# brucechin/OctopusZK

Hardware: AMD Instinct MI355X
Metric: BN254 G1 VariableBaseMSM Mscalar-mul/s at 2^20 (higher is better)
Workload: dtype u32; 1 GPU; VariableBaseMSM BN254 G1 2^20 random scalars/bases per GPU, bit-exact vs the serial CPU path (BASELINE.json configs[1]); n_per_gpu=1048576, window_bits=16, windows=8, glv=True, prepared_bases=False, msms_in_flight=3, schedule=pipeline3, parallelism=index-range shard x1, RCCL all-gather of 192-B partials + HIP point sum

## Files before the change

### octopuszk_amd/csrc/glv.cuh

```cuda
#pragma once
#include "curve.cuh"

namespace ozk {

struct GlvConsts {
  static constexpr u32 R32[8] = {0xf0000001u, 0x43e1f593u, 0x79b97091u, 0x2833e848u, 0x8181585du, 0xb85045b6u, 0xe131a029u, 0x30644e72u};
  static constexpr u32 G1C[3] = {0xc7e0b3d7u, 0xd91d232eu, 0x00000002u};
  static constexpr u32 G2C[5] = {0x391eb18du, 0x7a7bd9d4u, 0xa773d2cfu, 0x4ccef014u, 0x00000002u};
  static constexpr u32 A1[2] = {0x94d213e3u, 0x89d32568u};
  static constexpr u32 A2[4] = {0x1221250bu, 0x0be4e154u, 0xeeb859fdu, 0x6f4d8248u};
  static constexpr u32 B1ABS[4] = {0x7d4f1128u, 0x8211bbebu, 0xeeb859fcu, 0x6f4d8248u};
  static constexpr u32 B2[2] = {0x94d213e3u, 0x89d32568u};
  static constexpr u32 BETA_G1[9] = {0xa337995u, 0x158d1d23u, 0x189c9b98u, 0x12fa4e45u, 0x185faadcu, 0x176f16du, 0xeed93bau, 0x14291140u, 0xc0afeu};
  static constexpr u32 BETA_G2[9] = {0x18ccb791u, 0x175b1c3au, 0xb83d6e2u, 0xe8ed071u, 0x1282bee2u, 0x4220e84u, 0x1fe4017fu, 0x15084d4au, 0x169119u};
};

template <int NA, int NB, int NR>
OZK_HD void mp_mul_lo(const u32* a, const u32* b, u32* r) {
  u64 carry = 0;
#pragma unroll
  for (int k = 0; k < NR; k++) {
    u64 lo = carry & 0xffffffffull;
    u64 hi = carry >> 32;
#pragma unroll
    for (int i = 0; i < NA; i++) {
      const int j = k - i;
      if (j >= 0 && j < NB) {
        const u64 p = (u64)a[i] * b[j];
        lo += p & 0xffffffffull;
        hi += p >> 32;
      }
    }
    r[k] = (u32)lo;
    carry = hi + (lo >> 32);
  }
}
template <int NA, int NB>
OZK_HD void mp_mul(const u32* a, const u32* b, u32* r) { mp_mul_lo<NA, NB, NA + NB>(a, b, r); }

template <int N>
OZK_HD void mp_sub(u32* a, const u32* b) {
  u64 br = 0;
#pragma unroll
  for (int i = 0; i < N; i++) {
    const u64 t = (u64)a[i] - b[i] - br;
    a[i] = (u32)t;
    br = (t >> 32) & 1;
  }
}
template <int N>
OZK_HD bool mp_geq(const u32* a, const u32* b) {
  for (int i = N - 1; i >= 0; i--) {
    if (a[i] > b[i]) return true;
    if (a[i] < b[i]) return false;
  }
  return true;
}
template <int N>
OZK_HD void mp_neg(u32* a) {
  u64 c = 1;
#pragma unroll
  for (int i = 0; i < N; i++) {
    c += (u64)(~a[i]);
    a[i] = (u32)c;
    c >>= 32;
  }
}

OZK_HD void glv_decompose(const u32 (&k_in)[8], u32 (&k1)[4], bool& neg1, u32 (&k2)[4], bool& neg2) {
  u32 k[8];
#pragma unroll
  for (int i = 0; i < 8; i++) k[i] = k_in[i];
  for (int it = 0; it < 6 && mp_geq<8>(k, GlvConsts::R32); it++) mp_sub<8>(k, GlvConsts::R32);
  u32 p1[11], p2[13];
  mp_mul<8, 3>(k, GlvConsts::G1C, p1);
  mp_mul<8, 5>(k, GlvConsts::G2C, p2);
  const u32* c1 = p1 + 8;
  const u32* c2 = p2 + 8;
  u32 t1[5], t2[5], s1[5], s2[5];
  mp_mul_lo<3, 2, 5>(c1, GlvConsts::A1, t1);
  mp_mul_lo<5, 4, 5>(c2, GlvConsts::A2, t2);
#pragma unroll
  for (int i = 0; i < 5; i++) s1[i] = k[i];
  mp_sub<5>(s1, t1);
  mp_sub<5>(s1, t2);
  mp_mul_lo<3, 4, 5>(c1, GlvConsts::B1ABS, s2);
  mp_mul_lo<5, 2, 5>(c2, GlvConsts::B2, t2);
  mp_sub<5>(s2, t2);
  neg1 = (s1[4] >> 31) != 0;
  neg2 = (s2[4] >> 31) != 0;
  if (neg1) mp_neg<5>(s1);
  if (neg2) mp_neg<5>(s2);
#pragma unroll
  for (int i = 0; i < 4; i++) {
    k1[i] = s1[i];
    k2[i] = s2[i];
  }
}

template <class CV>
OZK_HD Fe<FqParams, 16> glv_beta() {
  if constexpr (CurveIO<CV>::CW == 16) return fe_const<FqParams, 16>(GlvConsts::BETA_G2);
  else return fe_const<FqParams, 16>(GlvConsts::BETA_G1);
}
template <class CV>
OZK_HD Aff<typename CV::EA> glv_image(const Aff<typename CV::EA>& q) {
  Aff<typename CV::EA> q2;
  q2.x = typename CV::EA(canonical(scale(q.x, glv_beta<CV>())));
  q2.y = q.y;
  return q2;
}

}
```

### octopuszk_amd/csrc/msm_var.cuh

```cuda
#pragma once
#include "curve.cuh"
#include "glv.cuh"

namespace ozk {

constexpr u32 BID_NONE = 0xffffffffu;

struct MsmPlan {
  int n_in;
  int glv;
  int n;
  int sd;
  int c;
  int cb;
  int W;
  int L1;
  int LK;
  int S;
};

OZK_HD u32 scalar_digit(const u32 (&s)[8], int w, int c) {
  const int bit = w * c;
  const int wi = bit >> 5, sh = bit & 31;
  u32 v = s[wi] >> sh;
  if (sh + c > 32 && wi + 1 < 8) v |= s[wi + 1] << (32 - sh);
  return v & ((1u << c) - 1u);
}

OZK_HD bool digit_decode(u32 code, int sd, u32& b, u32& neg) {
  if (sd) {
    const u32 t = code - 1u;
    b = t >> 1;
    neg = t & 1u;
  } else {
    b = code;
    neg = 0;
  }
  return code != 0;
}
template <class Emit>
OZK_HD void signed_digit_codes(const u32 (&e)[8], int c, int W, bool neg, Emit emit) {
  const u32 half = 1u << (c - 1);
  const u32 thr = (c == 16 && neg) ? half - 1u : half;
  u32 cy = 0;
  for (int w = 0; w < W; w++) {
    const u32 d = scalar_digit(e, w, c) + cy;
    cy = d > thr;
    const u32 m = cy ? (1u << c) - d : d;
    emit(w, (uint16_t)(m ? (((m - 1u) << 1) | (cy ^ (u32)neg)) + 1u : 0u));
  }
}

constexpr u32 SIDX_NEG = 0x80000000u;

#if defined(__HIPCC__)


template <class CV>
__global__ void __launch_bounds__(256) k_convert_bases(const u32* __restrict__ wire,
                                                       u32* __restrict__ aff, int n, int glv,
                                                       const uint8_t* __restrict__ neg_flags) {
  using IO = CurveIO<CV>;
  using EA = typename CV::EA;
  using ET = ElemTraits<EA>;
  const int i = blockIdx.x * blockDim.x + threadIdx.x;
  if (i >= n) return;
  const u32* p = wire + (size_t)i * IO::WIRE_JAC_WORDS;
  u32* o = aff + (size_t)i * IO::AFF_WORDS;
  Aff<EA> q;
  if (ET::wire_is_zero(p + 2 * IO::CW)) {
    q.x = EA(el_zero(q.x));
    q.y = EA(el_zero(q.x));
  } else if (ET::wire_is_one(p + 2 * IO::CW)) {
    q.x = ET::from_wire(p);
    q.y = ET::from_wire(p + IO::CW);
  } else {
    const EA X = ET::from_wire(p), Y = ET::from_wire(p + IO::CW), Z = ET::from_wire(p + 2 * IO::CW);
    const auto zi = inv(Z);
    if (is_zero(Z)) {
      q.x = EA(el_zero(q.x));
      q.y = EA(el_zero(q.x));
    } else {
      const auto zi2 = sqr(zi);
      q.x = EA(canonical(mul(X, zi2)));
      q.y = EA(canonical(mul(Y, mul(zi2, zi))));
    }
  }
  q.x = EA(canonical(q.x));
  q.y = EA(canonical(q.y));
  if (!glv) {
    IO::store_aff(q, o);
    return;
  }
  Aff<EA> q2;
  q2.x = EA(canonical(scale(q.x, glv_beta<CV>())));
  q2.y = q.y;
  if (neg_flags != nullptr) {
    const EA ny = EA(canonical(neg(q.y)));
    if (neg_flags[i]) q.y = ny;
    if (neg_flags[n + i]) q2.y = ny;
  }
  IO::store_aff(q, o);
  IO::store_aff(q2, aff + (size_t)(n + i) * IO::AFF_WORDS);
}

static __global__ void __launch_bounds__(256) k_digits(const u32* __restrict__ scalars, int n, int c, int W,
                                                uint16_t* __restrict__ digits) {
  const int i = blockIdx.x * blockDim.x + threadIdx.x;
  if (i >= n) return;
  u32 s[8];
  const uint4* sp = reinterpret_cast<const uint4*>(scalars + (size_t)i * 8);
  const uint4 a = sp[0], b = sp[1];
  s[0] = a.x; s[1] = a.y; s[2] = a.z; s[3] = a.w;
  s[4] = b.x; s[5] = b.y; s[6] = b.z; s[7] = b.w;
  for (int w = 0; w < W; w++) digits[(size_t)w * n + i] = (uint16_t)scalar_digit(s, w, c);
}

static __global__ void __launch_bounds__(256) k_digits_glv(const u32* __restrict__ scalars, int n, int c, int W, int sd,
                                                    uint16_t* __restrict__ digits, uint8_t* __restrict__ neg_flags) {
  const int i = blockIdx.x * blockDim.x + threadIdx.x;
  if (i >= n) return;
  u32 s[8];
  const uint4* sp = reinterpret_cast<const uint4*>(scalars + (size_t)i * 8);
  const uint4 a = sp[0], b = sp[1];
  s[0] = a.x; s[1] = a.y; s[2] = a.z; s[3] = a.w;
  s[4] = b.x; s[5] = b.y; s[6] = b.z; s[7] = b.w;
  u32 k1[4], k2[4];
  bool n1, n2;
  glv_decompose(s, k1, n1, k2, n2);
  u32 e1[8] = {k1[0], k1[1], k1[2], k1[3], 0, 0, 0, 0};
  u32 e2[8] = {k2[0], k2[1], k2[2], k2[3], 0, 0, 0, 0};
  const size_t ne = 2 * (size_t)n;
  if (sd) {
    signed_digit_codes(e1, c, W, n1, [&](int w, uint16_t code) { digits[(size_t)w * ne + i] = code; });
    signed_digit_codes(e2, c, W, n2, [&](int w, uint16_t code) { digits[(size_t)w * ne + n + i] = code; });
    return;
  } else {
    for (int w = 0; w < W; w++) {
      digits[(size_t)w * ne + i] = (uint16_t)scalar_digit(e1, w, c);
      digits[(size_t)w * ne + n + i] = (uint16_t)scalar_digit(e2, w, c);
    }
  }
  neg_flags[i] = n1;
  neg_flags[n + i] = n2;
}

constexpr int SORT_CHUNK = 4096;
constexpr int SORT_BLOCK = 256;

template <bool AGGREGATE = true>
__device__ __forceinline__ u32 lds_rank(u32* cnt, u32 key, bool live) {
  if constexpr (!AGGREGATE) return live ? atomicAdd(&cnt[key], 1u) : 0u;
  const unsigned long long m = __ballot(live);
  u32 r = 0;
  if (m != 0ull) {
    const int lane = threadIdx.x & 63;
    const int leader = __ffsll((long long)m) - 1;
    const u32 kl = __shfl(key, leader);
    if (__all(!live || key == kl)) {
      u32 base = 0;
      if (lane == leader) base = atomicAdd(&cnt[kl], (u32)__popcll(m));
      base = __shfl(base, leader);
      r = base + (u32)__popcll(m & ((1ull << lane) - 1ull));
    } else if (live) {
      r = atomicAdd(&cnt[key], 1u);
    }
  }
  return r;
}

static __global__ void __launch_bounds__(SORT_BLOCK) k_sort1_count(const uint16_t* __restrict__ digits, int n, int lo_bits,
                                                            int sd, int NH, int nblk, u32* __restrict__ C1) {
  extern __shared__ u32 cnt[];
  const int w = blockIdx.y, blk = blockIdx.x;
  for (int h = threadIdx.x; h < NH; h += SORT_BLOCK) cnt[h] = 0;
  block_sync();
  const int i0 = blk * SORT_CHUNK;
  constexpr int PER = SORT_CHUNK / SORT_BLOCK;
  u32 dreg[PER];
#pragma unroll
  for (int k = 0; k < PER; k++) {
    const int i = i0 + k * SORT_BLOCK + threadIdx.x;
    dreg[k] = (i < n) ? digits[(size_t)w * n + i] : 0u;
  }
#pragma unroll
  for (int k = 0; k < PER; k++) {
    u32 b, neg;
    const bool live = digit_decode(dreg[k], sd, b, neg);
    lds_rank(cnt, b >> lo_bits, live);
  }
  block_sync();
  for (int h = threadIdx.x; h < NH; h += SORT_BLOCK) C1[((size_t)w * NH + h) * nblk + blk] = cnt[h];
}

static __global__ void __launch_bounds__(SORT_BLOCK) k_sort1_scatter(const uint16_t* __restrict__ digits, int n, int lo_bits,
                                                              int sd, int NH, int nblk, const u32* __restrict__ P1,
                                                              const u32* __restrict__ total, size_t nC1,
                                                              u32* __restrict__ coarse) {
  extern __shared__ u32 sm[];
  u32* gdelta = sm;
  u32* lcur = sm + NH;
  u32* stage = sm + 2 * NH;
  u32* dest = stage + SORT_CHUNK;
  __shared__ u32 wsum[SORT_BLOCK / 64];
  __shared__ u32 n_local;
  const int w = blockIdx.y, blk = blockIdx.x;
  const int t = threadIdx.x;
  u32 g0 = 0, ct = 0;
  if (t < NH) {
    const size_t idx = ((size_t)w * NH + t) * nblk + blk;
    g0 = P1[idx];
    ct = ((idx + 1 < nC1) ? P1[idx + 1] : *total) - g0;
  }
  u32 incl = ct;
  const int lane = t & 63;
#pragma unroll
  for (int o = 1; o < 64; o <<= 1) {
    const u32 x = __shfl_up(incl, o);
    if (lane >= o) incl += x;
  }
// ... 733 lines not shown
        }
        cur = b;
        cur_cb = (p == s) && cb;
        if (b != BID_NONE) acc.start(pts_in, idx_in, p);
      } else if (b != BID_NONE) {
        acc.accumulate(pts_in, idx_in, p);
      }
    }
    }
    if (cur != BID_NONE) {
      if (cur_cb) {
        head_bid = cur;
        acc.store(pts_out + (size_t)(2 * (size_t)t) * IO::REC_WORDS);
        if (cf) {
          tail_bid = cur;
          if constexpr (FIRST) {
            acc.store_infinity(pts_out + (size_t)(2 * (size_t)t + 1) * IO::REC_WORDS);
          } else {
            IO::store_rec_jac(jac_infinity<CV>(), pts_out + (size_t)(2 * (size_t)t + 1) * IO::REC_WORDS);
          }
        }
      } else if (cf) {
        tail_bid = cur;
        acc.store(pts_out + (size_t)(2 * (size_t)t + 1) * IO::REC_WORDS);
      } else {
        acc.store(buckets + (size_t)cur * IO::REC_WORDS);
      }
    }
  }
  bid_out[2 * (size_t)t] = head_bid;
  bid_out[2 * (size_t)t + 1] = tail_bid;
}

template <class CV, bool FIRST, bool LAZY = false>
__global__ void __launch_bounds__(256, (FIRST && CV::LDS_ACC) ? 2 : 1)
k_segreduce(const u32* __restrict__ bid_in, const u32* __restrict__ idx_in, const u32* __restrict__ pts_in,
            const u32* __restrict__ d_count, int n_in_static, int L,
            u32* __restrict__ buckets, u32* __restrict__ bid_out, u32* __restrict__ pts_out,
            int n_lanes, unsigned long long* __restrict__ clk) {
  const int t = blockIdx.x * blockDim.x + threadIdx.x;
  unsigned long long w0 = 0, c0 = 0;
  if constexpr (FIRST) {
    if (clk != nullptr && threadIdx.x == 0) {
      w0 = (unsigned long long)wall_clock64();
      c0 = (unsigned long long)clock64();
      atomicMax(&clk[0], ~w0);
    }
  }
  if (t < n_lanes)
    segreduce_lane<CV, FIRST, LAZY>(t, bid_in, idx_in, pts_in, d_count, n_in_static, L, buckets, bid_out, pts_out);
  if constexpr (FIRST) {
    if (clk != nullptr && (threadIdx.x & 63) == 0) {
      const unsigned long long w1 = (unsigned long long)wall_clock64();
      atomicMax(&clk[1], w1);
      if (threadIdx.x == 0) {
        atomicAdd(&clk[2], (unsigned long long)clock64() - c0);
        atomicAdd(&clk[3], w1 - w0);
      }
    }
  }
}

static __global__ void k_read_clock(unsigned long long* out) { out[0] = (unsigned long long)wall_clock64(); }

template <class CV>
__global__ void __launch_bounds__(256)
k_segreduce_small(const u32* __restrict__ d_count, int n_in, int L, u32* __restrict__ buckets,
                  u32* __restrict__ bid_a, u32* __restrict__ pts_a, u32* __restrict__ bid_b, u32* __restrict__ pts_b) {
  if (*d_count == 0) return;
  u32 *bi = bid_a, *pi = pts_a, *bo = bid_b, *po = pts_b;
  while (true) {
    const int lanes = (n_in + L - 1) / L;
    for (int t = threadIdx.x; t < lanes; t += blockDim.x)
      segreduce_lane<CV, false>(t, bi, nullptr, pi, d_count, n_in, L, buckets, bo, po);
    if (lanes == 1) break;
    block_sync();
    n_in = 2 * lanes;
    u32* tb = bi; bi = bo; bo = tb;
    u32* tp = pi; pi = po; po = tp;
  }
}

constexpr int RUN_MAX = 16;
template <class CV>
__global__ void __launch_bounds__(256)
k_runmerge(const u32* __restrict__ bid_in, const u32* __restrict__ pts, int n_slots,
           u32* __restrict__ buckets, u32* __restrict__ bid_out, u32* __restrict__ remaining) {
  using IO = CurveIO<CV>;
  const int t = blockIdx.x * blockDim.x + threadIdx.x;
  u32 alive = 0;
#pragma unroll 1
  for (int k = 0; k < 2; k++) {
    const int x = 2 * t + 1 + k;
    if (x >= n_slots) break;
    const u32 bx = bid_in[x];
    u32 out = BID_NONE;
    if (bx != BID_NONE) {
      int s = x, e = x;
      while (s > 0 && x - s < RUN_MAX && bid_in[s - 1] == bx) s--;
      while (e + 1 < n_slots && e - x < RUN_MAX && bid_in[e + 1] == bx) e++;
      const bool is_short = (x - s < RUN_MAX) && (e - x < RUN_MAX) && (e - s + 1 <= RUN_MAX);
      if (!is_short) {
        out = bx;
      } else if (s == x) {
        Xyzz<CV> acc = IO::load_xyzz(pts + (size_t)s * IO::REC_WORDS);
        for (int q = s + 1; q <= e; q += 2) acc = xyzz_add(acc, IO::load_xyzz(pts + (size_t)q * IO::REC_WORDS));
        IO::store_rec_xyzz(acc, buckets + (size_t)bx * IO::REC_WORDS);
      }
    }
    bid_out[x] = out;
    alive += (out != BID_NONE);
  }
  if (t == 0 && n_slots > 0) {
    bid_out[0] = bid_in[0];
    alive += (bid_in[0] != BID_NONE);
  }
  for (int o = 32; o > 0; o >>= 1) alive += __shfl_xor(alive, o);
  if ((threadIdx.x & 63) == 0 && alive) atomicAdd(remaining, alive);
}

template <class CV, bool FIRSTLEVEL>
__global__ void __launch_bounds__(256)
k_wsum(const u32* __restrict__ A_in, const u32* __restrict__ R_in, const u32* __restrict__ hist,
       int m_in, int S, int g, u32* __restrict__ A_out, u32* __restrict__ R_out, int m_out, int W, int prio) {
  using IO = CurveIO<CV>;
  if (prio) __builtin_amdgcn_s_setprio(3);
  const int t = blockIdx.x * blockDim.x + threadIdx.x;
  if (t >= m_out * W) return;
  const int w = t / m_out, j = t - w * m_out;
  const size_t base = (size_t)w * m_in;
  const int lo = j * S;
  int hi = lo + S;
  if (hi > m_in) hi = m_in;
  Jac<CV> run = jac_infinity<CV>(), ws = jac_infinity<CV>(), asum = jac_infinity<CV>();
  for (int e = hi - 1; e >= lo; e--) {
    if constexpr (FIRSTLEVEL) {
      if (hist[base + e] != 0) run = jac_add(run, IO::load_rec(R_in + (base + e) * IO::REC_WORDS));
    } else {
      run = jac_add(run, IO::load_jac(R_in + (base + e) * IO::JAC_WORDS));
    }
    if (e > lo) ws = jac_add(ws, run);
    if constexpr (!FIRSTLEVEL) asum = jac_add(asum, IO::load_jac(A_in + (base + e) * IO::JAC_WORDS));
  }
  for (int k = 0; k < g; k++) ws = jac_dbl(ws);
  if constexpr (!FIRSTLEVEL) ws = jac_add(ws, asum);
  IO::store_jac(ws, A_out + ((size_t)w * m_out + j) * IO::JAC_WORDS);
  IO::store_jac(run, R_out + ((size_t)w * m_out + j) * IO::JAC_WORDS);
}

template <class CV>
__device__ __forceinline__ Jac<CV> shfl_down_jac(const Jac<CV>& p, int o) {
  Jac<CV> r;
  r.X = shfl_down_el(p.X, o);
  r.Y = shfl_down_el(p.Y, o);
  r.Z = shfl_down_el(p.Z, o);
  return r;
}

template <class CV>
__device__ __forceinline__ void wave_combine(Jac<CV>& A, Jac<CV>& T, int l, int valid, int g) {
  for (int o = 1; o < valid; o <<= 1) {
    const Jac<CV> t = shfl_down_jac(T, o);
    const Jac<CV> s = jac_add(T, t);
    if (l + o < 64) T = s;
  }
  Jac<CV> U = T;
  for (int k = 0; k < g; k++) U = jac_dbl(U);
  const Jac<CV> AV = jac_add(A, U);
  Jac<CV> V = (l >= 1) ? AV : A;
  int top = 1;
  while (top < valid) top <<= 1;
  for (int o = top >> 1; o > 0; o >>= 1) {
    const Jac<CV> v = shfl_down_jac(V, o);
    const Jac<CV> s = jac_add(V, v);
    if (l < o) V = s;
  }
  A = V;
}

template <class CV>
__global__ void __launch_bounds__(64)
k_wsum_wave(const u32* __restrict__ A_in, const u32* __restrict__ R_in, int m_in, int g,
            u32* __restrict__ A_out, u32* __restrict__ R_out, int m_out, int W) {
  using IO = CurveIO<CV>;
  __builtin_amdgcn_s_setprio(3);
  const int wave = blockIdx.x;
  if (wave >= m_out * W) return;
  const int w = wave / m_out, j = wave - w * m_out;
  const int l = threadIdx.x & 63;
  const int e = j * 64 + l;
  int valid = m_in - j * 64;
  if (valid > 64) valid = 64;
  Jac<CV> A = jac_infinity<CV>(), T = jac_infinity<CV>();
  if (e < m_in) {
    A = IO::load_jac(A_in + ((size_t)w * m_in + e) * IO::JAC_WORDS);
    T = IO::load_jac(R_in + ((size_t)w * m_in + e) * IO::JAC_WORDS);
  }
  wave_combine<CV>(A, T, l, valid, g);
  if (l == 0) {
    IO::store_jac(A, A_out + ((size_t)w * m_out + j) * IO::JAC_WORDS);
    IO::store_jac(T, R_out + ((size_t)w * m_out + j) * IO::JAC_WORDS);
// ... 220 lines not shown
```

### octopuszk_amd/csrc/msm_var_driver.cuh

```cuda
#pragma once
#include <hip/hip_ext.h>
#include <pthread.h>
#include <stdlib.h>

#include <atomic>
#include <vector>

#ifndef OZK_WITH_G2
#define OZK_WITH_G2 1
#endif
#include "msm_var.cuh"
#include "host_ctx.h"
#include "fq2.cuh"

namespace ozk {

enum { PROF_OFF = 0, PROF_EVENTS = 1, PROF_CLOCK = 2 };
struct ProfState {
  pthread_mutex_t mu = PTHREAD_MUTEX_INITIALIZER;
  std::atomic<int> mode{PROF_OFF};
  int src = PROF_EVENTS;
  int every = 1, seen = 0;
  int count = 0;
  std::vector<hipEvent_t> e0, e1;
// ... 212 lines not shown
}
template <class CV>
RegionBytes region_bytes(int n) {
  RegionBytes rb;
  make_layout3<CV>(plan_for<CV>(n), nullptr, nullptr, nullptr, &rb);
  return rb;
}

template <class CV>
size_t tail_layout(const MsmPlan& p, MsmLayout& L, void* tail, size_t tail_bytes) {
  using IO = CurveIO<CV>;
  Bump b(tail, tail_bytes);
  L.NB = (size_t)p.W << p.cb;
  L.m1 = (((size_t)1 << p.cb) + p.S - 1) / p.S;
  L.buckets = b.take<u32>(L.NB * IO::REC_WORDS);
  L.hist_t = b.take<u32>(L.NB);
  for (int k = 0; k < 2; k++) {
    L.wA[k] = b.take<u32>((size_t)p.W * L.m1 * IO::JAC_WORDS);
    L.wR[k] = b.take<u32>((size_t)p.W * L.m1 * IO::JAC_WORDS);
  }
  b.take<u32>(64);
  return b.off;
}

enum { TAIL_LATENCY = 0, TAIL_THROUGHPUT = 1 };
struct TailShape {
  bool fused;
  int serial_above;
};
static TailShape tail_shape(int mode) {
  const int forced = env_int("OZK_MSM_TAIL_MODE", -1);
  if (forced == 0 || forced == 1) mode = forced;
  TailShape t;
  t.fused = env_int("OZK_MSM_WSUM_FUSED", mode == TAIL_THROUGHPUT ? 0 : 1) != 0;
  t.serial_above = env_int("OZK_MSM_TAIL_SERIAL_ABOVE", mode == TAIL_THROUGHPUT ? 64 : (1 << 30));
  return t;
}
static void first_level_shape(const MsmPlan& p, bool fused, int* m_out, int* g_out) {
  const int m_in = 1 << p.cb;
  const int nseg = (m_in + p.S - 1) / p.S;
  const int sg = ilog2((uint32_t)p.S);
  if (fused) {
    *m_out = (nseg + 63) / 64;
    *g_out = sg + 6;
  } else {
    *m_out = nseg;
    *g_out = sg;
  }
}
template <class CV>
void launch_wsum0(const MsmPlan& p, const MsmLayout& L, hipStream_t st, int prio, bool fused) {
  const int TB = 256;
  const int m_in = 1 << p.cb;
  int m_out, g;
  first_level_shape(p, fused, &m_out, &g);
  const int tot = m_out * p.W;
  if (fused)
    hipLaunchKernelGGL((k_wsum_fused<CV>), dim3(tot), dim3(64), 0, st, L.buckets, L.hist_t, m_in, p.S,
                       ilog2((uint32_t)p.S), L.wA[0], L.wR[0], m_out, p.W, prio);
  else
    hipLaunchKernelGGL((k_wsum<CV, true>), dim3((tot + TB - 1) / TB), dim3(TB), 0, st, (const u32*)nullptr,
                       L.buckets, L.hist_t, m_in, p.S, 0, L.wA[0], L.wR[0], m_out, p.W, prio);
}

template <class CV>
int var_msm_sort(const void* d_bases, const void* d_scalars, int n, void* sorted, size_t sorted_bytes,
                        void* sort_ws, size_t sort_ws_bytes, hipStream_t st, hipEvent_t order_ev = nullptr,
                        const void* prepared = nullptr) {
  hip_clear_stale();
  const MsmPlan p = plan_for<CV>(n);
  if (prepared && p.glv && !p.sd) return fail(OZK_E_INVALID, "prepared bases need the signed-digit plan");
  RegionBytes rb;
  const MsmLayout L = make_layout3<CV>(p, sorted, sort_ws, nullptr, &rb, prepared);
  if (rb.sorted > sorted_bytes || rb.sort_ws > sort_ws_bytes)
    return fail(OZK_E_INVALID, "sort buffers too small: need %zu + %zu bytes, got %zu + %zu", rb.sorted, rb.sort_ws,
                sorted_bytes, sort_ws_bytes);
  const int TB = 256;
  const u32* bases = (const u32*)d_bases;
  const u32* scalars = (const u32*)d_scalars;
  const int n_in = p.n_in;
  n = p.n;
  OZK_HIP(hipMemsetAsync(L.total, 0, 4 * sizeof(u32), st));
  if (p.glv) {
    hipLaunchKernelGGL(k_digits_glv, dim3((n_in + TB - 1) / TB), dim3(TB), 0, st, scalars, n_in, p.c, p.W, p.sd,
                       L.digits, L.neg_flags);
    if (!prepared)
      hipLaunchKernelGGL((k_convert_bases<CV>), dim3((n_in + TB - 1) / TB), dim3(TB), 0, st, bases, L.aff, n_in, 1,
                         p.sd ? (const uint8_t*)nullptr : (const uint8_t*)L.neg_flags);
  } else {
    if (!prepared)
      hipLaunchKernelGGL((k_convert_bases<CV>), dim3((n_in + TB - 1) / TB), dim3(TB), 0, st, bases, L.aff, n_in, 0,
                         (const uint8_t*)nullptr);
    hipLaunchKernelGGL(k_digits, dim3((n_in + TB - 1) / TB), dim3(TB), 0, st, scalars, n_in, p.c, p.W, L.digits);
  }
  if (n <= SORTS_MAX_N && p.cb <= SORTS_MAX_CB && env_int("OZK_MSM_SMALL_SORT", 1)) {
    hipLaunchKernelGGL(k_sort_small, dim3(p.W), dim3(SORTS_BLOCK), 0, st, L.digits, n, p.cb, p.sd, L.total, L.hist, L.sent);
    if (order_ev && env_int("OZK_MSM_ORDER", 1)) OZK_HIP(hipStreamWaitEvent(st, order_ev, 0));
    OZK_HIP(hipGetLastError());
    return OZK_OK;
  }
  const size_t lds1 = (size_t)L.NH * sizeof(u32);
  hipLaunchKernelGGL(k_sort1_count, dim3(L.nblk, p.W), dim3(SORT_BLOCK), lds1, st, L.digits, n, L.lo_bits, p.sd,
                     L.NH, L.nblk, L.C1);
  const int items = SCAN_BLOCK * SCAN_ITEMS;
  const int nb = (int)((L.nC1 + items - 1) / items);
  hipLaunchKernelGGL(k_scan_blocksum, dim3(nb), dim3(SCAN_BLOCK), 0, st, L.C1, (int)L.nC1, L.blocksum);
  hipLaunchKernelGGL(k_scan_top, dim3(1), dim3(1024), 0, st, L.blocksum, nb, L.total);
  hipLaunchKernelGGL(k_scan_final, dim3(nb), dim3(SCAN_BLOCK), 0, st, L.C1, (int)L.nC1, L.blocksum, L.P1);
  const size_t lds_sc = ((size_t)2 * L.NH + 2 * SORT_CHUNK) * sizeof(u32);
  hipLaunchKernelGGL(k_sort1_scatter, dim3(L.nblk, p.W), dim3(SORT_BLOCK), lds_sc, st, L.digits, n, L.lo_bits,
                     p.sd, L.NH, L.nblk, L.P1, L.total, L.nC1, L.coarse);
  const int nbins = p.W * L.NH;
  const u32 sign_bit = p.sd ? 0x80u : 0u;
  const u32 big_thresh = (u32)(n / 64) > SORT_BIG ? (u32)(n / 64) : SORT_BIG;
  if (L.cap / ((size_t)big_thresh + 1) > (size_t)SORTBIG_MAXBINS)
    return fail(OZK_E_INVALID, "window plan c=%d (W=%d) at n=%d can produce more than %d oversized sort bins",
                p.c, p.W, p.n_in, SORTBIG_MAXBINS);
  hipLaunchKernelGGL(k_sort2, dim3(nbins), dim3(SORT2_BLOCK), 0, st, L.coarse, L.P1, L.total, p.cb, L.lo_bits, L.NH,
                     sign_bit, L.nblk, nbins, big_thresh, L.hist, L.sent);
  if (order_ev && env_int("OZK_MSM_ORDER", 1)) OZK_HIP(hipStreamWaitEvent(st, order_ev, 0));
  hipLaunchKernelGGL(k_sortbig_list, dim3(1), dim3(256), 0, st, L.P1, L.total, L.nblk, nbins, big_thresh, L.bigbins);
  hipLaunchKernelGGL(k_sortbig_count, dim3(1024), dim3(SORT_BLOCK), 0, st, L.coarse, L.bigbins,
                     (1u << L.lo_bits) - 1u, L.bigT);
  hipLaunchKernelGGL(k_sortbig_scan, dim3(SORTBIG_MAXBINS), dim3(256), 0, st, L.bigbins, L.bigT, p.cb, L.lo_bits, L.NH,
                     L.hist);
  hipLaunchKernelGGL(k_sortbig_scatter, dim3(1024), dim3(SORT_BLOCK), 0, st, L.coarse, L.bigbins, L.bigT, p.cb,
                     L.lo_bits, sign_bit, L.NH, L.sent);
  OZK_HIP(hipGetLastError());
  return OZK_OK;
}

enum { ACCUM_ALL = 0, ACCUM_LEVEL1 = 1, ACCUM_REST = 2 };
template <class CV>
int var_msm_accum(int n, void* sorted, size_t sorted_bytes, void* accum_ws, size_t accum_ws_bytes, void* tail,
                         size_t tail_bytes, hipStream_t st, const void* prepared = nullptr, int part = ACCUM_ALL) {
  hip_clear_stale();
  using CT = CV;
  const MsmPlan p = plan_for<CV>(n);
  RegionBytes rb;
  MsmLayout L = make_layout3<CV>(p, sorted, nullptr, accum_ws, &rb, prepared);
  if (rb.sorted > sorted_bytes || rb.accum_ws > accum_ws_bytes)
    return fail(OZK_E_INVALID, "accumulate buffers too small: need %zu + %zu bytes, got %zu + %zu", rb.sorted,
                rb.accum_ws, sorted_bytes, accum_ws_bytes);
  const size_t tneed = tail_layout<CV>(p, L, tail, tail_bytes);
  if (tneed > tail_bytes) return fail(OZK_E_INVALID, "tail buffer too small: need %zu bytes, got %zu", tneed, tail_bytes);
  const int TB = 256;
  size_t lanes = (L.cap + p.L1 - 1) / p.L1;
  if (part != ACCUM_REST) {
  hipEvent_t prof_e0 = nullptr, prof_e1 = nullptr;
  unsigned long long* clk = nullptr;
  g_prof.claim(&prof_e0, &prof_e1, &clk);
  const bool prof = prof_e0 != nullptr;
  size_t acc_lds = CV::LDS_ACC ? (size_t)RunAccLds<CV>::LDS_WORDS * TB * sizeof(u32) : 0;
  if (!CV::LDS_ACC) acc_lds = (size_t)env_int("OZK_L1_LDS", 41216);
  auto launch_l1 = [&](auto kern) {
    if (acc_lds > 65536)
      OZK_HIP(hipFuncSetAttribute((const void*)kern, hipFuncAttributeMaxDynamicSharedMemorySize, (int)acc_lds));
    hipExtLaunchKernelGGL(kern, dim3((unsigned)((lanes + TB - 1) / TB)), dim3(TB), (uint32_t)acc_lds, st,
                          prof ? prof_e0 : (hipEvent_t) nullptr, prof ? prof_e1 : (hipEvent_t) nullptr, 0u,
                          (const u32*)nullptr, (const u32*)L.sent, (const u32*)L.aff, (const u32*)L.total, 0, p.L1,
                          L.buckets, L.slot_bid[0], L.slot_pts[0], (int)lanes, clk);
    return OZK_OK;
  };
  int rc_l1;
  if constexpr (CV::LAZY_MADD) {
    if (env_int("OZK_L1_LAZY", 1)) rc_l1 = launch_l1(k_segreduce<CV, true, true>);
    else rc_l1 = launch_l1(k_segreduce<CV, true, false>);
  } else {
    rc_l1 = launch_l1(k_segreduce<CV, true, false>);
  }
  if (rc_l1) return rc_l1;
  }
  if (part == ACCUM_LEVEL1) {
    OZK_HIP(hipGetLastError());
    return OZK_OK;
// ... 170 lines not shown
    OZK_HIP(hipMemsetAsync(d_bases + (size_t)n * base_rec, 0, (padded - n) * base_rec, up));
  }
  const MsmPlan p = plan_for<CV>(per);
  SliceBuckets sb = {};
  for (int s = 0; s < K; s++) {
    const size_t lo = (size_t)s * per;
    const size_t ns = ((size_t)n - lo < (size_t)per) ? ((size_t)n - lo) : (size_t)per;
    if (scalars && (rc = staged_h2d(c, d_sc + lo * 32, scalars + lo * 32, ns * 32, up))) return rc;
    if ((rc = staged_h2d(c, d_bases + lo * base_rec, bases + lo * base_rec, ns * base_rec, up))) return rc;
    OZK_HIP(hipEventRecord(ev[s], up));
    OZK_HIP(hipStreamWaitEvent(st, ev[s], 0));
    uint8_t* tail = d_tails + (size_t)s * tb;
    const int n_head = (s == K - 1 && exact_last) ? (int)last_ns : per;
    if ((rc = var_msm_head<CV>(d_bases + lo * base_rec, d_sc + lo * 32, n_head, d_ws, main_bytes, tail, tb, st))) return rc;
    MsmLayout L;
    tail_layout<CV>(p, L, tail, tb);
    sb.buckets[s] = L.buckets;
    sb.hist[s] = L.hist_t;
  }
  const size_t NB = (size_t)p.W << p.cb;
  hipLaunchKernelGGL((k_bucket_combine<CV>), dim3((unsigned)((NB + 255) / 256)), dim3(256), 0, st, sb, K,
                     (u32*)sb.buckets[0], (u32*)sb.hist[0], NB);
  OZK_HIP(hipGetLastError());
  return var_msm_tail<CV>(per, d_tails, tb, d_out, st);
}

inline int host_result(HostCtx* c, uint8_t* out, uint8_t* d_result, const uint8_t* d_out, size_t bytes, hipStream_t st) {
  if (!d_result) return staged_d2h(c, out, d_out, bytes, st);
  OZK_HIP(hipMemcpyAsync(d_result, d_out, bytes, hipMemcpyDeviceToDevice, st));
  StatTimer tm(host_call_stats().sync_ms);
  OZK_HIP(hipStreamSynchronize(st));
  return OZK_OK;
}

template <class CV>
int var_msm_host(const uint8_t* bases, const uint8_t* scalars, int n, int task_id, uint8_t* out,
                 uint8_t* d_result = nullptr) {
  using IO = CurveIO<CV>;
  CtxGuard g;
  int rc = ctx_acquire(task_id, &g.c);
  if (rc) return rc;
  HostCtx* c = g.c;
  const size_t base_rec = (size_t)IO::WIRE_JAC_WORDS * 4;
  const size_t out_bytes = (size_t)IO::WIRE_JAC_WORDS * 8;
  const int K = host_slices(n);
  if (K == 1) {
    const size_t base_bytes = (size_t)n * base_rec, sc_bytes = (size_t)n * 32;
    const size_t ws_bytes = var_msm_ws_bytes<CV>(n);
    if ((rc = ctx_reserve(c, pad256(base_bytes) + pad256(sc_bytes) + 1024 + ws_bytes + 1024))) return rc;
    uint8_t* d_bases = c->arena;
    uint8_t* d_sc = d_bases + pad256(base_bytes);
    uint8_t* d_out = d_sc + pad256(sc_bytes);
    uint8_t* d_ws = d_out + 1024;
    hipStream_t st = c->st[0];
    if ((rc = staged_h2d(c, d_sc, scalars, sc_bytes, st))) return rc;
    if ((rc = staged_h2d(c, d_bases, bases, base_bytes, st))) return rc;
    if ((rc = var_msm_dev<CV>(d_bases, d_sc, n, d_out, d_ws, ws_bytes, st))) return rc;
    return host_result(c, out, d_result, d_out, out_bytes, st);
  }
  const int per = host_slice_per(n, K);
  const size_t padded = (size_t)K * per;
  if ((rc = ctx_reserve(c, pad256(padded * base_rec) + pad256(padded * 32) + 1024 + host_sliced_ws_bytes<CV>(K, per) + 1024)))
    return rc;
  uint8_t* d_bases = c->arena;
  uint8_t* d_sc = d_bases + pad256(padded * base_rec);
  uint8_t* d_out = d_sc + pad256(padded * 32);
  uint8_t* d_ws = d_out + 1024;
  if ((rc = host_sliced_msm<CV>(c, bases, scalars, n, K, per, d_bases, d_sc, d_ws, d_out, c->slice_ev, c->st[0], c->st[2])))
    return rc;
  return host_result(c, out, d_result, d_out, out_bytes, c->st[0]);
}

template <class CV>
size_t prepared_bytes(int n) {
  const MsmPlan p = plan_for<CV>(n);
  return (((size_t)p.n * CurveIO<CV>::AFF_WORDS * sizeof(u32)) + 255) & ~(size_t)255;
}
template <class CV>
int var_msm_prepare(const void* d_bases, int n, void* d_prepared, size_t bytes, hipStream_t st) {
  hip_clear_stale();
  const MsmPlan p = make_plan(n);
  if (p.glv && !p.sd) return fail(OZK_E_INVALID, "prepared bases need the signed-digit plan");
  if (bytes < prepared_bytes<CV>(n)) return fail(OZK_E_INVALID, "prepared buffer too small");
  hipLaunchKernelGGL((k_convert_bases<CV>), dim3((n + 255) / 256), dim3(256), 0, st, (const u32*)d_bases,
                     (u32*)d_prepared, n, p.glv, (const uint8_t*)nullptr);
  OZK_HIP(hipGetLastError());
  return OZK_OK;
}

constexpr uint32_t BASES_MAGIC = 0x4f5a4b42u;
struct BasesHandle {
  uint32_t magic;
  int refs;
  int device, n, type;
  hipStream_t st;
  uint8_t *d_prepared, *d_scalars, *d_out, *d_ws;
  uint8_t* h_out;
  size_t ws_bytes;
  pthread_mutex_t mu;
};

template <class CV>
int bases_create(const uint8_t* bases, int n, int type, int task_id, BasesHandle** out) {
  using IO = CurveIO<CV>;
  int rc = select_device(task_id);
  if (rc) return rc;
  BasesHandle* h = (BasesHandle*)calloc(1, sizeof(BasesHandle));
  if (!h) return fail(OZK_E_NOMEM, "out of host memory");
  hipGetDevice(&h->device);
  h->n = n;
  h->type = type == OZK_G1 ? OZK_G1 : OZK_G2;
  pthread_mutex_init(&h->mu, nullptr);
  const size_t wire = (size_t)n * IO::WIRE_JAC_WORDS * 4, pb = prepared_bytes<CV>(n);
  h->ws_bytes = var_msm_ws_bytes<CV>(n);
  hipError_t e = hipStreamCreateWithFlags(&h->st, hipStreamNonBlocking);
  uint8_t* d_wire = nullptr;
  if (e == hipSuccess) e = hipMalloc((void**)&h->d_prepared, pb);
  if (e == hipSuccess) e = hipMalloc((void**)&h->d_scalars, (size_t)n * 32 + 256);
  if (e == hipSuccess) e = hipMalloc((void**)&h->d_out, 1024);
  if (e == hipSuccess) e = hipHostMalloc((void**)&h->h_out, 1024, hipHostMallocDefault);
  if (e == hipSuccess) e = hipMalloc((void**)&h->d_ws, h->ws_bytes);
  if (e == hipSuccess) e = hipMalloc((void**)&d_wire, wire);
  rc = OZK_OK;
  if (e == hipSuccess) {
    CtxGuard g;
    rc = ctx_acquire(task_id, &g.c);
    if (!rc) rc = staged_h2d(g.c, d_wire, bases, wire, h->st);
    if (!rc) e = hipStreamSynchronize(h->st);
  }
  if (e == hipSuccess && !rc) rc = var_msm_prepare<CV>(d_wire, n, h->d_prepared, pb, h->st);
  if (e == hipSuccess && !rc) e = hipStreamSynchronize(h->st);
  if (d_wire) hipFree(d_wire);
  if (e != hipSuccess || rc) {
    if (h->d_prepared) hipFree(h->d_prepared);
    if (h->d_scalars) hipFree(h->d_scalars);
    if (h->d_out) hipFree(h->d_out);
    if (h->h_out) hipHostFree(h->h_out);
    if (h->d_ws) hipFree(h->d_ws);
    if (h->st) hipStreamDestroy(h->st);
    free(h);
    if (rc) return rc;
    return fail(OZK_E_NOMEM, "HIP failure while preparing bases: %s", hipGetErrorString(e));
  }
  h->magic = BASES_MAGIC;
  *out = h;
  return OZK_OK;
}

template <class CV>
int bases_msm(BasesHandle* h, const uint8_t* scalars, uint8_t* out) {
  const size_t out_bytes = (size_t)CurveIO<CV>::WIRE_JAC_WORDS * 8;
  pthread_mutex_lock(&h->mu);
  if (h->magic != BASES_MAGIC) {
    pthread_mutex_unlock(&h->mu);
    return fail(OZK_E_INVALID, "bases handle was released");
  }
  int rc = OZK_OK;
  hipError_t e = hipSetDevice(h->device);
  do {
    if (e != hipSuccess) break;
    {
      CtxGuard g;
      rc = ctx_acquire(h->device, &g.c);
      if (!rc) rc = staged_h2d(g.c, h->d_scalars, scalars, (size_t)h->n * 32, h->st);
      if (!rc) e = hipStreamSynchronize(h->st);
    }
    if (rc || e != hipSuccess) break;
// ... 33 lines not shown
```

Baseline: 712.1 Mscalar-mul/s.

## Speed up GLV digit prep, base conversion, and parallelize run-merge walks

Several independent changes. GLV scalar reduction now uses a single quotient estimate plus one conditional subtract, replacing the loop of up to six compare-and-subtract passes, and the multiprecision multiply switches to row-wise carry accumulation. Digit extraction gets a compile-time window-16 specialization with unrolled loops over the 128-bit half scalars. Base conversion drops redundant canonicalization and turns the neg-flag branch into a template parameter. The run-merge kernel finds run boundaries with wavefront shuffles and prefix scans instead of per-thread linear walks, and spreads long short-run accumulations across threads through an LDS work list; this adds shared-memory and sync overhead, and the correctness of the run-ownership logic is a risk.

```diff
diff --git a/octopuszk_amd/csrc/glv.cuh b/octopuszk_amd/csrc/glv.cuh
--- a/octopuszk_amd/csrc/glv.cuh
+++ b/octopuszk_amd/csrc/glv.cuh
@@ -5,6 +5,7 @@
 
 struct GlvConsts {
   static constexpr u32 R32[8] = {0xf0000001u, 0x43e1f593u, 0x79b97091u, 0x2833e848u, 0x8181585du, 0xb85045b6u, 0xe131a029u, 0x30644e72u};
+  static constexpr u32 NEG_R32[8] = {0x0fffffffu, 0xbc1e0a6cu, 0x86468f6eu, 0xd7cc17b7u, 0x7e7ea7a2u, 0x47afba49u, 0x1ece5fd6u, 0xcf9bb18du};
   static constexpr u32 G1C[3] = {0xc7e0b3d7u, 0xd91d232eu, 0x00000002u};
   static constexpr u32 G2C[5] = {0x391eb18du, 0x7a7bd9d4u, 0xa773d2cfu, 0x4ccef014u, 0x00000002u};
   static constexpr u32 A1[2] = {0x94d213e3u, 0x89d32568u};
@@ -17,22 +18,20 @@
 
 template <int NA, int NB, int NR>
 OZK_HD void mp_mul_lo(const u32* a, const u32* b, u32* r) {
-  u64 carry = 0;
 #pragma unroll
-  for (int k = 0; k < NR; k++) {
-    u64 lo = carry & 0xffffffffull;
-    u64 hi = carry >> 32;
+  for (int k = 0; k < NR; k++) r[k] = 0;
+#pragma unroll
+  for (int j = 0; j < NB; j++) {
+    u32 carry = 0;
 #pragma unroll
     for (int i = 0; i < NA; i++) {
-      const int j = k - i;
-      if (j >= 0 && j < NB) {
-        const u64 p = (u64)a[i] * b[j];
-        lo += p & 0xffffffffull;
-        hi += p >> 32;
+      if (i + j < NR) {
+        const u64 t = (u64)a[i] * b[j] + r[i + j] + carry;
+        r[i + j] = (u32)t;
+        carry = (u32)(t >> 32);
       }
     }
-    r[k] = (u32)lo;
-    carry = hi + (lo >> 32);
+    if (j + NA < NR) r[j + NA] = carry;
   }
 }
 template <int NA, int NB>
@@ -67,11 +66,32 @@
   }
 }
 
+OZK_HD void mp_reduce_r(u32 (&k)[8]) {
+  const u32 q = k[7] / (GlvConsts::R32[7] + 1u);
+  u32 carry = 0;
+#pragma unroll
+  for (int i = 0; i < 8; i++) {
+    const u64 t = (u64)q * GlvConsts::NEG_R32[i] + k[i] + carry;
+    k[i] = (u32)t;
+    carry = (u32)(t >> 32);
+  }
+  u32 d[8];
+  u64 br = 0;
+#pragma unroll
+  for (int i = 0; i < 8; i++) {
+    const u64 t = (u64)k[i] - GlvConsts::R32[i] - br;
+    d[i] = (u32)t;
+    br = (t >> 32) & 1;
+  }
+#pragma unroll
+  for (int i = 0; i < 8; i++) k[i] = br ? k[i] : d[i];
+}
+
 OZK_HD void glv_decompose(const u32 (&k_in)[8], u32 (&k1)[4], bool& neg1, u32 (&k2)[4], bool& neg2) {
   u32 k[8];
 #pragma unroll
   for (int i = 0; i < 8; i++) k[i] = k_in[i];
-  for (int it = 0; it < 6 && mp_geq<8>(k, GlvConsts::R32); it++) mp_sub<8>(k, GlvConsts::R32);
+  mp_reduce_r(k);
   u32 p1[11], p2[13];
   mp_mul<8, 3>(k, GlvConsts::G1C, p1);
   mp_mul<8, 5>(k, GlvConsts::G2C, p2);
diff --git a/octopuszk_amd/csrc/msm_var.cuh b/octopuszk_amd/csrc/msm_var.cuh
--- a/octopuszk_amd/csrc/msm_var.cuh
+++ b/octopuszk_amd/csrc/msm_var.cuh
@@ -51,12 +51,36 @@
   }
 }
 
+template <int C>
+OZK_HD u32 half_scalar_digit(const u32 (&s)[4], int w) {
+  static_assert(C >= 1 && C <= 16, "window bits");
+  const int bit = w * C;
+  const int wi = bit >> 5, sh = bit & 31;
+  u32 v = s[wi] >> sh;
+  if (sh + C > 32 && wi + 1 < 4) v |= s[wi + 1] << (32 - sh);
+  return v & ((1u << C) - 1u);
+}
+template <int C, class Emit>
+OZK_HD void signed_digit_codes_ct(const u32 (&e)[4], bool neg, Emit emit) {
+  constexpr int W = (128 + C - 1) / C;
+  constexpr u32 half = 1u << (C - 1);
+  const u32 thr = (C == 16 && neg) ? half - 1u : half;
+  u32 cy = 0;
+#pragma unroll
+  for (int w = 0; w < W; w++) {
+    const u32 d = half_scalar_digit<C>(e, w) + cy;
+    cy = d > thr;
+    const u32 m = cy ? (1u << C) - d : d;
+    emit(w, (uint16_t)(m ? (((m - 1u) << 1) | (cy ^ (u32)neg)) + 1u : 0u));
+  }
+}
+
 constexpr u32 SIDX_NEG = 0x80000000u;
 
 #if defined(__HIPCC__)
 
 
-template <class CV>
+template <class CV, bool NEGF>
 __global__ void __launch_bounds__(256) k_convert_bases(const u32* __restrict__ wire,
                                                        u32* __restrict__ aff, int n, int glv,
                                                        const uint8_t* __restrict__ neg_flags) {
@@ -72,8 +96,8 @@
     q.x = EA(el_zero(q.x));
     q.y = EA(el_zero(q.x));
   } else if (ET::wire_is_one(p + 2 * IO::CW)) {
-    q.x = ET::from_wire(p);
-    q.y = ET::from_wire(p + IO::CW);
+    q.x = EA(canonical(ET::from_wire(p)));
+    q.y = EA(canonical(ET::from_wire(p + IO::CW)));
   } else {
     const EA X = ET::from_wire(p), Y = ET::from_wire(p + IO::CW), Z = ET::from_wire(p + 2 * IO::CW);
     const auto zi = inv(Z);
@@ -86,8 +110,6 @@
       q.y = EA(canonical(mul(Y, mul(zi2, zi))));
     }
   }
-  q.x = EA(canonical(q.x));
-  q.y = EA(canonical(q.y));
   if (!glv) {
     IO::store_aff(q, o);
     return;
@@ -95,7 +117,7 @@
   Aff<EA> q2;
   q2.x = EA(canonical(scale(q.x, glv_beta<CV>())));
   q2.y = q.y;
-  if (neg_flags != nullptr) {
+  if constexpr (NEGF) {
     const EA ny = EA(canonical(neg(q.y)));
     if (neg_flags[i]) q.y = ny;
     if (neg_flags[n + i]) q2.y = ny;
@@ -116,6 +138,7 @@
   for (int w = 0; w < W; w++) digits[(size_t)w * n + i] = (uint16_t)scalar_digit(s, w, c);
 }
 
+template <int C>
 static __global__ void __launch_bounds__(256) k_digits_glv(const u32* __restrict__ scalars, int n, int c, int W, int sd,
                                                     uint16_t* __restrict__ digits, uint8_t* __restrict__ neg_flags) {
   const int i = blockIdx.x * blockDim.x + threadIdx.x;
@@ -128,14 +151,27 @@
   u32 k1[4], k2[4];
   bool n1, n2;
   glv_decompose(s, k1, n1, k2, n2);
-  u32 e1[8] = {k1[0], k1[1], k1[2], k1[3], 0, 0, 0, 0};
-  u32 e2[8] = {k2[0], k2[1], k2[2], k2[3], 0, 0, 0, 0};
   const size_t ne = 2 * (size_t)n;
-  if (sd) {
-    signed_digit_codes(e1, c, W, n1, [&](int w, uint16_t code) { digits[(size_t)w * ne + i] = code; });
-    signed_digit_codes(e2, c, W, n2, [&](int w, uint16_t code) { digits[(size_t)w * ne + n + i] = code; });
-    return;
+  if constexpr (C != 0) {
+    constexpr int WC = (128 + C - 1) / C;
+    if (sd) {
+      signed_digit_codes_ct<C>(k1, n1, [&](int w, uint16_t code) { digits[(size_t)w * ne + i] = code; });
+      signed_digit_codes_ct<C>(k2, n2, [&](int w, uint16_t code) { digits[(size_t)w * ne + n + i] = code; });
+      return;
+    }
+#pragma unroll
+    for (int w = 0; w < WC; w++) {
+      digits[(size_t)w * ne + i] = (uint16_t)half_scalar_digit<C>(k1, w);
+      digits[(size_t)w * ne + n + i] = (uint16_t)half_scalar_digit<C>(k2, w);
+    }
   } else {
+    u32 e1[8] = {k1[0], k1[1], k1[2], k1[3], 0, 0, 0, 0};
+    u32 e2[8] = {k2[0], k2[1], k2[2], k2[3], 0, 0, 0, 0};
+    if (sd) {
+      signed_digit_codes(e1, c, W, n1, [&](int w, uint16_t code) { digits[(size_t)w * ne + i] = code; });
+      signed_digit_codes(e2, c, W, n2, [&](int w, uint16_t code) { digits[(size_t)w * ne + n + i] = code; });
+      return;
+    }
     for (int w = 0; w < W; w++) {
       digits[(size_t)w * ne + i] = (uint16_t)scalar_digit(e1, w, c);
       digits[(size_t)w * ne + n + i] = (uint16_t)scalar_digit(e2, w, c);
@@ -1035,41 +1071,114 @@
 }
 
 constexpr int RUN_MAX = 16;
+constexpr u32 RUNM_FROM_PTS = 0x80000000u;
 template <class CV>
 __global__ void __launch_bounds__(256)
 k_runmerge(const u32* __restrict__ bid_in, const u32* __restrict__ pts, int n_slots,
-           u32* __restrict__ buckets, u32* __restrict__ bid_out, u32* __restrict__ remaining) {
+           u32* buckets, u32* __restrict__ bid_out, u32* __restrict__ remaining) {
   using IO = CurveIO<CV>;
+  __shared__ u32 lst_n;
+  __shared__ u32 lst_q[256], lst_e[256], lst_b[256];
+  if (threadIdx.x == 0) lst_n = 0;
+  block_sync();
   const int t = blockIdx.x * blockDim.x + threadIdx.x;
+  const int lane = threadIdx.x & 63;
+  const int x = 2 * t + 1, y = x + 1;
+  const u32 bx = x < n_slots ? bid_in[x] : BID_NONE;
+  const u32 by = y < n_slots ? bid_in[y] : BID_NONE;
+  u32 prev = __shfl_up(by, 1), next = __shfl_down(bx, 1);
+  if (lane == 0) prev = x - 1 < n_slots ? bid_in[x - 1] : BID_NONE;
+  if (lane == 63) next = y + 1 < n_slots ? bid_in[y + 1] : BID_NONE;
+  const bool sx = bx != prev, sy = by != bx, ey = by != next;
+  int vs = sy ? y : (sx ? x : -1);
+  int ve = sy ? x : (ey ? y : 0x7fffffff);
+#pragma unroll
+  for (int o = 1; o < 64; o <<= 1) {
+    const int us = __shfl_up(vs, o), ue = __shfl_down(ve, o);
+    if (lane >= o) vs = max(vs, us);
+    if (lane + o < 64) ve = min(ve, ue);
+  }
+  const int vs_before = __shfl_up(vs, 1), ve_after = __shfl_down(ve, 1);
+  int s_x = sx ? x : (lane > 0 ? vs_before : -1), s_y = vs;
+  int e_x = ve, e_y = ey ? y : (lane < 63 ? ve_after : 0x7fffffff);
+  const int w_first = 2 * (t - lane) + 1, w_last = w_first + 127;
+  auto walk_left = [&](int i, u32 b) {
+    int s = w_first;
+    while (s > 0 && i - s < RUN_MAX && bid_in[s - 1] == b) s--;
+    return s;
+  };
+  auto walk_right = [&](int i, u32 b) {
+    int e = w_last;
+    while (e + 1 < n_slots && e - i < RUN_MAX && bid_in[e + 1] == b) e++;
+    return e;
+  };
+  auto is_short = [](int i, int s, int e) {
+    return (i - s < RUN_MAX) && (e - i < RUN_MAX) && (e - s + 1 <= RUN_MAX);
+  };
+  bool short_x = false, short_y = false;
+  if (bx != BID_NONE) {
+    if (s_x < 0) s_x = walk_left(x, bx);
+    if (e_x == 0x7fffffff) e_x = walk_right(x, bx);
+    short_x = is_short(x, s_x, e_x);
+  }
+  if (by != BID_NONE) {
+    if (s_y < 0) s_y = walk_left(y, by);
+    if (e_y == 0x7fffffff) e_y = walk_right(y, by);
+    short_y = is_short(y, s_y, e_y);
+  }
+  const u32 out_x = (bx != BID_NONE && !short_x) ? bx : BID_NONE;
+  const u32 out_y = (by != BID_NONE && !short_y) ? by : BID_NONE;
   u32 alive = 0;
-#pragma unroll 1
-  for (int k = 0; k < 2; k++) {
-    const int x = 2 * t + 1 + k;
-    if (x >= n_slots) break;
-    const u32 bx = bid_in[x];
-    u32 out = BID_NONE;
-    if (bx != BID_NONE) {
-      int s = x, e = x;
-      while (s > 0 && x - s < RUN_MAX && bid_in[s - 1] == bx) s--;
-      while (e + 1 < n_slots && e - x < RUN_MAX && bid_in[e + 1] == bx) e++;
-      const bool is_short = (x - s < RUN_MAX) && (e - x < RUN_MAX) && (e - s + 1 <= RUN_MAX);
-      if (!is_short) {
-        out = bx;
-      } else if (s == x) {
-        Xyzz<CV> acc = IO::load_xyzz(pts + (size_t)s * IO::REC_WORDS);
-        for (int q = s + 1; q <= e; q += 2) acc = xyzz_add(acc, IO::load_xyzz(pts + (size_t)q * IO::REC_WORDS));
-        IO::store_rec_xyzz(acc, buckets + (size_t)bx * IO::REC_WORDS);
-      }
-    }
-    bid_out[x] = out;
-    alive += (out != BID_NONE);
+  if (x < n_slots) {
+    bid_out[x] = out_x;
+    alive += (out_x != BID_NONE);
+  }
+  if (y < n_slots) {
+    bid_out[y] = out_y;
+    alive += (out_y != BID_NONE);
   }
   if (t == 0 && n_slots > 0) {
     bid_out[0] = bid_in[0];
     alive += (bid_in[0] != BID_NONE);
   }
+  const bool own_x = short_x && s_x == x;
+  const bool own_y = short_y && s_y == y;
+  const bool more_x = own_x && e_x >= x + 3;
+  const bool listed = more_x || own_y;
+  const unsigned long long lm = __ballot(listed);
+  u32 lpos = 0;
+  if (lm != 0ull) {
+    const int leader = __ffsll((long long)lm) - 1;
+    if (lane == leader) lpos = atomicAdd(&lst_n, (u32)__popcll(lm));
+    lpos = __shfl(lpos, leader) + (u32)__popcll(lm & ((1ull << lane) - 1ull));
+  }
+  if (own_x) {
+    Xyzz<CV> acc = IO::load_xyzz(pts + (size_t)x * IO::REC_WORDS);
+    if (e_x > x) acc = xyzz_add(acc, IO::load_xyzz(pts + (size_t)y * IO::REC_WORDS));
+    IO::store_rec_xyzz(acc, buckets + (size_t)bx * IO::REC_WORDS);
+    if (more_x) {
+      lst_q[lpos] = (u32)(x + 3);
+      lst_e[lpos] = (u32)e_x;
+      lst_b[lpos] = bx;
+    }
+  }
+  if (own_y) {
+    lst_q[lpos] = (u32)(y + 1);
+    lst_e[lpos] = (u32)e_y | RUNM_FROM_PTS;
+    lst_b[lpos] = by;
+  }
+  block_sync();
+  if (threadIdx.x < lst_n) {
+    u32 q = lst_q[threadIdx.x];
+    const u32 el = lst_e[threadIdx.x], b = lst_b[threadIdx.x];
+    const u32 e = el & ~RUNM_FROM_PTS;
+    const u32* src = (el & RUNM_FROM_PTS) ? pts + (size_t)(q - 1) * IO::REC_WORDS : buckets + (size_t)b * IO::REC_WORDS;
+    Xyzz<CV> acc = IO::load_xyzz(src);
+    for (; q <= e; q += 2) acc = xyzz_add(acc, IO::load_xyzz(pts + (size_t)q * IO::REC_WORDS));
+    IO::store_rec_xyzz(acc, buckets + (size_t)b * IO::REC_WORDS);
+  }
   for (int o = 32; o > 0; o >>= 1) alive += __shfl_xor(alive, o);
-  if ((threadIdx.x & 63) == 0 && alive) atomicAdd(remaining, alive);
+  if (lane == 0 && alive) atomicAdd(remaining, alive);
 }
 
 template <class CV, bool FIRSTLEVEL>
diff --git a/octopuszk_amd/csrc/msm_var_driver.cuh b/octopuszk_amd/csrc/msm_var_driver.cuh
--- a/octopuszk_amd/csrc/msm_var_driver.cuh
+++ b/octopuszk_amd/csrc/msm_var_driver.cuh
@@ -318,15 +318,24 @@
   n = p.n;
   OZK_HIP(hipMemsetAsync(L.total, 0, 4 * sizeof(u32), st));
   if (p.glv) {
-    hipLaunchKernelGGL(k_digits_glv, dim3((n_in + TB - 1) / TB), dim3(TB), 0, st, scalars, n_in, p.c, p.W, p.sd,
-                       L.digits, L.neg_flags);
-    if (!prepared)
-      hipLaunchKernelGGL((k_convert_bases<CV>), dim3((n_in + TB - 1) / TB), dim3(TB), 0, st, bases, L.aff, n_in, 1,
-                         p.sd ? (const uint8_t*)nullptr : (const uint8_t*)L.neg_flags);
+    if (p.c == 16 && p.W == 8)
+      hipLaunchKernelGGL(k_digits_glv<16>, dim3((n_in + TB - 1) / TB), dim3(TB), 0, st, scalars, n_in, p.c, p.W, p.sd,
+                         L.digits, L.neg_flags);
+    else
+      hipLaunchKernelGGL(k_digits_glv<0>, dim3((n_in + TB - 1) / TB), dim3(TB), 0, st, scalars, n_in, p.c, p.W, p.sd,
+                         L.digits, L.neg_flags);
+    if (!prepared) {
+      if (p.sd)
+        hipLaunchKernelGGL((k_convert_bases<CV, false>), dim3((n_in + TB - 1) / TB), dim3(TB), 0, st, bases, L.aff, n_in,
+                           1, (const uint8_t*)nullptr);
+      else
+        hipLaunchKernelGGL((k_convert_bases<CV, true>), dim3((n_in + TB - 1) / TB), dim3(TB), 0, st, bases, L.aff, n_in,
+                           1, (const uint8_t*)L.neg_flags);
+    }
   } else {
     if (!prepared)
-      hipLaunchKernelGGL((k_convert_bases<CV>), dim3((n_in + TB - 1) / TB), dim3(TB), 0, st, bases, L.aff, n_in, 0,
-                         (const uint8_t*)nullptr);
+      hipLaunchKernelGGL((k_convert_bases<CV, false>), dim3((n_in + TB - 1) / TB), dim3(TB), 0, st, bases, L.aff, n_in,
+                         0, (const uint8_t*)nullptr);
     hipLaunchKernelGGL(k_digits, dim3((n_in + TB - 1) / TB), dim3(TB), 0, st, scalars, n_in, p.c, p.W, L.digits);
   }
   if (n <= SORTS_MAX_N && p.cb <= SORTS_MAX_CB && env_int("OZK_MSM_SMALL_SORT", 1)) {
@@ -663,7 +672,7 @@
   const MsmPlan p = make_plan(n);
   if (p.glv && !p.sd) return fail(OZK_E_INVALID, "prepared bases need the signed-digit plan");
   if (bytes < prepared_bytes<CV>(n)) return fail(OZK_E_INVALID, "prepared buffer too small");
-  hipLaunchKernelGGL((k_convert_bases<CV>), dim3((n + 255) / 256), dim3(256), 0, st, (const u32*)d_bases,
+  hipLaunchKernelGGL((k_convert_bases<CV, false>), dim3((n + 255) / 256), dim3(256), 0, st, (const u32*)d_bases,
                      (u32*)d_prepared, n, p.glv, (const uint8_t*)nullptr);
   OZK_HIP(hipGetLastError());
   return OZK_OK;
```

New measurement: 726.5 Mscalar-mul/s (median of 6 runs). 2.0% higher.
